# 92MING/Stable-Renderer

Hardware: AMD Instinct MI355X
Metric: frames/sec @512^2, SD1.5 20-step img2img, 8-view overlap (higher is better)
Workload: dtype f16

## Files before the change

include/sr_hip.h:

```cpp
#ifndef SR_HIP_H
#define SR_HIP_H
#include <stdint.h>
#ifdef __cplusplus
extern "C" {
#endif

typedef enum {
  SR_OK = 0,
  SR_ERR_INVALID = -1,
  SR_ERR_LAUNCH = -2,
  SR_ERR_UNSUPPORTED = -3
} sr_status;

typedef enum { SR_F16 = 0, SR_F32 = 1 } sr_dtype;

const char* sr_last_error(void);
int sr_version(void);
const char* sr_source_hash(void);
int sr_device_sync(void);

typedef struct {
  const void* a;
  const void* a2;
  const void* w;
  const float* bias;
  const float* rowvec;
  const void* residual;
  void* out;
  const void* zero_page;
  int32_t B, H, W;
  int32_t C1, C2;
  int32_t N;
  int32_t KH;
  int32_t stride;
  int32_t upsample;
  int32_t act;
  int32_t transpose_out;
  int32_t ldt;
  int32_t out_f32;
  int32_t dtype;
  float scale;
  int32_t rowvec_ld;
  void* workspace;
  int64_t workspace_bytes;
  const float* row_stats;
  const float* colsum;
  int32_t tile;
  int32_t split;
  int32_t pad_br;
  const void* prefetch;
  int64_t prefetch_bytes;
  int32_t up_h, up_w;
  int32_t* split_counters;
  int32_t group;
  int32_t ln_inline;
  float ln_eps;
  int32_t tile_order;
} sr_igemm_args;
#define SR_IGEMM_SPLIT_COUNTERS 4096
#define SR_IGEMM_GROUP_MAX 4
int sr_igemm(const sr_igemm_args* args, void* stream);
int sr_igemm_group(const sr_igemm_args* const* args, int32_t n, void* stream);

typedef struct {
  const void* x; const void* x2;
  const float* gamma; const float* beta;
  void* y;
  float* partials;
  int32_t B, HW, C1, C2, groups, silu, dtype;
  float eps;
} sr_groupnorm_args;
int sr_groupnorm(const sr_groupnorm_args* args, void* stream);
int64_t sr_groupnorm_scratch_floats(int32_t B, int32_t HW);

int sr_row_stats(const void* x, float* stats, int32_t rows, int32_t C, float eps, int32_t dtype, void* stream);
int sr_layernorm(const void* x, const float* gamma, const float* beta, void* y, int32_t rows, int32_t C,
                 float eps, int32_t dtype, void* stream);
int sr_layernorm_gather(const void* x, const int32_t* sel, int32_t nsel, int32_t frame_rows, int32_t n_frames, int32_t* err_flag,
                        const float* gamma, const float* beta, void* y, int32_t C, float eps, int32_t dtype, void* stream);

typedef struct {
  const void* q; const void* k; const void* vt; void* o;
  int32_t B, Bk, Tq, Tk, heads, d, ldt, dtype;
  int32_t q_stride, k_stride;
  float scale;
} sr_attention_args;
int sr_attention(const sr_attention_args* args, void* stream);

int sr_nchw_to_nhwc(const float* x, void* y, int32_t B, int32_t C, int32_t HW, int32_t Cpad, float scale_mul,
                    const float* per_batch_scale, int32_t dtype, void* stream);
int sr_nhwc_to_nchw(const void* x, float* y, int32_t B, int32_t C, int32_t HW, int32_t ldc, int32_t dtype,
                    void* stream);
int sr_timestep_embedding(const float* t, void* y, int32_t B, int32_t dim, int32_t dtype, void* stream);
int sr_silu(const void* x, void* y, int64_t n, int32_t dtype, void* stream);
int sr_cast(const void* x, int32_t src_dtype, void* y, int32_t dst_dtype, int64_t n, void* stream);
int sr_cache_touch(const void* p, int64_t bytes, void* stream);
int sr_softmax_rows(void* x, int32_t rows, int32_t cols, int32_t dtype, void* stream);
int sr_gather_rows(const void* x, const int32_t* sel, void* y, int32_t nsel, int32_t n_rows, int64_t row_bytes,
                   int32_t* err_flag, void* stream);
int sr_add_scaled(const void* a, const void* b, void* y, int64_t n, float s, int32_t dtype, void* stream);

typedef enum {
  SR_OP_IGEMM = 1, SR_OP_GROUPNORM = 2, SR_OP_LAYERNORM = 3, SR_OP_ATTENTION = 4, SR_OP_NCHW_TO_NHWC = 5,
  SR_OP_NHWC_TO_NCHW = 6, SR_OP_TIMESTEP_EMBED = 7, SR_OP_SILU = 8, SR_OP_SOFTMAX_ROWS = 9, SR_OP_GATHER_ROWS = 10, SR_OP_ADD_SCALED = 11,
  SR_OP_FORK = 12,
  SR_OP_JOIN = 13,
  SR_OP_ROW_STATS = 14,
  SR_OP_LAYERNORM_GATHER = 15
} sr_op_kind;
typedef struct {
  int32_t kind; int32_t lane;
  union {
    sr_igemm_args igemm;
    sr_groupnorm_args gn;
    sr_attention_args attn;
    struct { const void* x; const float* gamma; const float* beta; void* y; int32_t rows, C, dtype; float eps;
             const int32_t* sel; int32_t* err_flag; int32_t frame_rows, n_frames; } ln;
    struct { const void* x; void* y; const float* per_batch_scale; int32_t B, C, HW, Cpad, dtype, ldc; float scale; } cvt;
    struct { const float* t; void* y; int32_t B, dim, dtype; } temb;
    struct { const void* x; void* y; int64_t n; int32_t dtype; int32_t rows, cols; } ew;
    struct { const void* x; void* y; const int32_t* sel; int64_t row_bytes; int32_t nsel; int32_t n_rows; int32_t* err_flag; } gather;
    struct { const void* a; const void* b; void* y; int64_t n; float s; int32_t dtype; } add;
  } u;
} sr_op;
int sr_plan_run(const sr_op* host_ops, int32_t n_ops, void* stream);
int sr_plan_capture(const sr_op* host_ops, int32_t n_ops, void* stream, void** graph_exec);
int sr_graph_launch(void* graph_exec, void* stream);
int sr_graph_destroy(void* graph_exec);

typedef struct sr_model sr_model;
int sr_model_load(const char* path, sr_model** model);
int sr_model_free(sr_model* model);
int sr_model_io(sr_model* model, const char* name, void** dev_ptr, int64_t* nbytes);
int sr_model_run(sr_model* model, const char* plan, void* stream);
int sr_model_write(sr_model* model, const char* name, const void* src, void* stream);
int sr_model_read(sr_model* model, const char* name, void* dst, void* stream);
int sr_unet_forward(sr_model* unet, const float* x, const float* t, const void* ctx, float* out, void* stream);
int sr_vae_decode(sr_model* vae, const float* z, float* img, void* stream);

int sr_eps_scale_input(const float* x, float* xin, int64_t n_per_copy, int32_t copies, float sigma, void* stream);
int sr_cfg_denoise(const float* x, const float* eps, float* denoised, float* d, int64_t n, int32_t copies,
                   float sigma, float cfg, void* stream);
int sr_cond_crop_scale(const float* x, float* xin, int32_t N, int32_t C, int32_t h, int32_t w, int32_t ah, int32_t aw, int32_t y0,
                       int32_t x0, int32_t chunks, float sigma, void* stream);
int sr_cond_accumulate(const float* x, const float* eps, const float* mult, const int32_t* kinds, float* out_c, float* cnt_c,
// ... 88 lines not shown
```

stable-renderer_amd/_lib.py:

```python
import ctypes as C
import os

_HERE = os.path.dirname(os.path.abspath(__file__))
LIB_PATH = os.path.join(_HERE, "csrc", "libsr_hip.so")
_DEV_LIB = os.environ.get("SR_DEV_LIB")

SR_F16, SR_F32 = 0, 1
(OP_IGEMM, OP_GROUPNORM, OP_LAYERNORM, OP_ATTENTION, OP_NCHW_TO_NHWC, OP_NHWC_TO_NCHW, OP_TIMESTEP_EMBED, OP_SILU,
 OP_SOFTMAX_ROWS, OP_GATHER_ROWS, OP_ADD_SCALED, OP_FORK, OP_JOIN, OP_ROW_STATS, OP_LAYERNORM_GATHER) = range(1, 16)

vp = C.c_void_p
i32 = C.c_int32
i64 = C.c_int64
f32 = C.c_float


class IgemmArgs(C.Structure):
    _fields_ = [("a", vp), ("a2", vp), ("w", vp), ("bias", vp), ("rowvec", vp), ("residual", vp), ("out", vp),
                ("zero_page", vp), ("B", i32), ("H", i32), ("W", i32), ("C1", i32), ("C2", i32), ("N", i32),
                ("KH", i32), ("stride", i32), ("upsample", i32), ("act", i32), ("transpose_out", i32), ("ldt", i32),
                ("out_f32", i32), ("dtype", i32), ("scale", f32), ("rowvec_ld", i32), ("workspace", vp),
                ("workspace_bytes", C.c_int64), ("row_stats", vp), ("colsum", vp), ("tile", i32), ("split", i32), ("pad_br", i32),
                ("prefetch", vp), ("prefetch_bytes", C.c_int64), ("up_h", i32), ("up_w", i32), ("split_counters", vp), ("group", i32), ("ln_inline", i32), ("ln_eps", f32), ("tile_order", i32)]


class GroupNormArgs(C.Structure):
    _fields_ = [("x", vp), ("x2", vp), ("gamma", vp), ("beta", vp), ("y", vp), ("partials", vp), ("B", i32),
                ("HW", i32), ("C1", i32), ("C2", i32), ("groups", i32), ("silu", i32), ("dtype", i32), ("eps", f32)]


class AttentionArgs(C.Structure):
    _fields_ = [("q", vp), ("k", vp), ("vt", vp), ("o", vp), ("B", i32), ("Bk", i32), ("Tq", i32), ("Tk", i32),
                ("heads", i32), ("d", i32), ("ldt", i32), ("dtype", i32), ("q_stride", i32), ("k_stride", i32),
                ("scale", f32)]


class _Ln(C.Structure):
    _fields_ = [("x", vp), ("gamma", vp), ("beta", vp), ("y", vp), ("rows", i32), ("C", i32), ("dtype", i32), ("eps", f32),
                ("sel", vp), ("err_flag", vp), ("frame_rows", i32), ("n_frames", i32)]


class _Cvt(C.Structure):
    _fields_ = [("x", vp), ("y", vp), ("per_batch_scale", vp), ("B", i32), ("C", i32), ("HW", i32), ("Cpad", i32),
                ("dtype", i32), ("ldc", i32), ("scale", f32)]


class _Temb(C.Structure):
    _fields_ = [("t", vp), ("y", vp), ("B", i32), ("dim", i32), ("dtype", i32)]


class _Ew(C.Structure):
    _fields_ = [("x", vp), ("y", vp), ("n", i64), ("dtype", i32), ("rows", i32), ("cols", i32)]


class _Gather(C.Structure):
    _fields_ = [("x", vp), ("y", vp), ("sel", vp), ("row_bytes", i64), ("nsel", i32), ("n_rows", i32), ("err_flag", vp)]


class _Add(C.Structure):
    _fields_ = [("a", vp), ("b", vp), ("y", vp), ("n", i64), ("s", f32), ("dtype", i32)]


class _OpU(C.Union):
    _fields_ = [("igemm", IgemmArgs), ("gn", GroupNormArgs), ("attn", AttentionArgs), ("ln", _Ln), ("cvt", _Cvt),
                ("temb", _Temb), ("ew", _Ew), ("gather", _Gather), ("add", _Add)]


class Op(C.Structure):
    _fields_ = [("kind", i32), ("lane", i32), ("u", _OpU)]


class Draw(C.Structure):
    _fields_ = [("pos", vp), ("normal", vp), ("uv", vp), ("color", vp), ("vertex_id", vp), ("tris", vp), ("nv", i32),
                ("nt", i32), ("MV", f32 * 16), ("MV_IT", f32 * 16), ("P", f32 * 16), ("sprite_id", i32),
                ("material_id", i32), ("corrmap_k", i32), ("use_texcoord_id", i32), ("render_mode", i32),
                ("has_vertex_color", i32), ("depth_test", i32), ("cull_back", i32), ("id_w", i32), ("id_h", i32),
                ("noise_tex", vp), ("noise_w", i32), ("noise_h", i32), ("diffuse_tex", vp), ("diffuse_w", i32),
                ("diffuse_h", i32), ("corrmap_tex", vp), ("corr_w", i32), ("corr_h", i32),
                ("tangent", vp), ("bitangent", vp), ("normal_tex", vp), ("normal_w", i32), ("normal_h", i32), ("diffuse_levels", i32)]


class GBuffer(C.Structure):
    _fields_ = [("color", vp), ("id", vp), ("pos", vp), ("normal_depth", vp), ("noise", vp), ("canny", vp), ("zbuf", vp),
                ("W", i32), ("H", i32)]


P = C.POINTER
SYMBOLS = {
    "sr_last_error": (C.c_char_p, []),
    "sr_version": (C.c_int, []),
    "sr_source_hash": (C.c_char_p, []),
    "sr_device_sync": (C.c_int, []),
    "sr_model_load": (C.c_int, [C.c_char_p, P(vp)]),
    "sr_model_free": (C.c_int, [vp]),
    "sr_model_io": (C.c_int, [vp, C.c_char_p, P(vp), P(i64)]),
    "sr_model_run": (C.c_int, [vp, C.c_char_p, vp]),
    "sr_model_write": (C.c_int, [vp, C.c_char_p, vp, vp]),
    "sr_model_read": (C.c_int, [vp, C.c_char_p, vp, vp]),
    "sr_unet_forward": (C.c_int, [vp, vp, vp, vp, vp, vp]),
    "sr_vae_decode": (C.c_int, [vp, vp, vp, vp]),
    "sr_layernorm_gather": (C.c_int, [vp, vp, i32, i32, i32, vp, vp, vp, vp, i32, f32, i32, vp]),
    "sr_igemm": (C.c_int, [P(IgemmArgs), vp]),
    "sr_igemm_group": (C.c_int, [P(P(IgemmArgs)), i32, vp]),
    "sr_groupnorm": (C.c_int, [P(GroupNormArgs), vp]),
    "sr_groupnorm_scratch_floats": (i64, [i32, i32]),
    "sr_layernorm": (C.c_int, [vp, vp, vp, vp, i32, i32, f32, i32, vp]),
    "sr_row_stats": (C.c_int, [vp, vp, i32, i32, f32, i32, vp]),
    "sr_attention": (C.c_int, [P(AttentionArgs), vp]),
    "sr_nchw_to_nhwc": (C.c_int, [vp, vp, i32, i32, i32, i32, f32, vp, i32, vp]),
    "sr_nhwc_to_nchw": (C.c_int, [vp, vp, i32, i32, i32, i32, i32, vp]),
    "sr_timestep_embedding": (C.c_int, [vp, vp, i32, i32, i32, vp]),
    "sr_silu": (C.c_int, [vp, vp, i64, i32, vp]),
    "sr_cast": (C.c_int, [vp, i32, vp, i32, i64, vp]),
    "sr_cache_touch": (C.c_int, [vp, i64, vp]),
    "sr_softmax_rows": (C.c_int, [vp, i32, i32, i32, vp]),
    "sr_gather_rows": (C.c_int, [vp, vp, vp, i32, i32, i64, vp, vp]),
    "sr_add_scaled": (C.c_int, [vp, vp, vp, i64, f32, i32, vp]),
    "sr_plan_run": (C.c_int, [P(Op), i32, vp]),
    "sr_plan_capture": (C.c_int, [P(Op), i32, vp, P(vp)]),
    "sr_graph_launch": (C.c_int, [vp, vp]),
    "sr_graph_destroy": (C.c_int, [vp]),
    "sr_eps_scale_input": (C.c_int, [vp, vp, i64, i32, f32, vp]),
    "sr_cfg_denoise": (C.c_int, [vp, vp, vp, vp, i64, i32, f32, f32, vp]),
    "sr_cond_crop_scale": (C.c_int, [vp, vp, i32, i32, i32, i32, i32, i32, i32, i32, i32, f32, vp]),
    "sr_cond_accumulate": (C.c_int, [vp, vp, vp, vp, vp, vp, vp, vp, i32, i32, i32, i32, i32, i32, i32, i32, i32, f32, vp]),
    "sr_cfg_combine": (C.c_int, [vp, vp, vp, vp, vp, vp, vp, i64, f32, f32, vp]),
    "sr_euler_step": (C.c_int, [vp, vp, i64, f32, vp]),
    "sr_vae_sample": (C.c_int, [vp, vp, vp, i32, i32, i32, vp]),
    "sr_ddpm_step": (C.c_int, [vp, vp, vp, i64, f32, f32, vp]),
    "sr_lcm_step": (C.c_int, [vp, vp, vp, i64, f32, vp]),
    "sr_axpby": (C.c_int, [vp, vp, i64, f32, f32, vp]),
    "sr_idmap_masks": (C.c_int, [vp, vp, i64, vp]),
    "sr_overlap_build": (C.c_int, [vp, i32, i32, i32, i32, i32, vp, vp, vp, vp]),
    "sr_overlap_csr_scratch_ints": (i64, [i32]),
    "sr_overlap_csr": (C.c_int, [vp, vp, i32, i32, i32, i32, vp, vp, vp, vp]),
    "sr_overlap_step": (C.c_int, [vp, vp, vp, vp, i32, i32, i32, i32, i32, f32, vp, vp]),
    "sr_legacy_overlap": (C.c_int, [vp, vp, vp, vp, vp, vp, vp, vp, i32, i32, i32, i32, i32, i32, f32, i32, i32, i32, vp]),
    "sr_legacy_levels": (C.c_int, [vp, vp, vp, vp, vp, i32, i32, i32, i32, i32, vp, vp]),
    "sr_legacy_overlap_seq": (C.c_int, [vp, vp, vp, vp, i32, i32, vp, vp, vp, vp, vp, i32, i32, i32, f32, i32, i32, vp]),
    "sr_nearest_resize": (C.c_int, [vp, vp, i64, i32, i32, i32, i32, vp, vp]),
    "sr_adain": (C.c_int, [vp, i64, i64, i64, i32, vp, i32, i64, i64, i64, i32, vp, i32, i32, f32, vp, vp]),
    "sr_noise_pool": (C.c_int, [vp, vp, vp, vp, vp, i32, i32, vp, vp]),
    "sr_noise_pool_strips": (C.c_int, [vp, vp, vp, vp, vp, i32, i32, i32, vp, vp]),
    "sr_corrmap_update": (C.c_int, [vp, i32, vp, vp, vp, i32, i32, i32, i32, i32, i32, vp, vp, i32, i32, vp, vp, vp]),
    "sr_gbuffer_clear": (C.c_int, [P(GBuffer), vp]),
    "sr_gbuffer_depth_merge": (C.c_int, [P(GBuffer), P(GBuffer), vp]),
    "sr_defer_post": (C.c_int, [vp, vp, vp, i32, i32, i32, i32, i32, f32, f32, f32, f32, f32, vp]),
    "sr_raster_draw": (C.c_int, [P(Draw), P(GBuffer), vp, i64, vp]),
    "sr_raster_scratch_bytes": (i64, [i32, i32, i32]),
}

_lib = None


class SrHipError(RuntimeError):
    pass


def _build_module():
    import importlib.util
    spec = importlib.util.spec_from_file_location("sr_build", os.path.join(_HERE, "csrc", "build.py"))
    mod = importlib.util.module_from_spec(spec)
    spec.loader.exec_module(mod)
    return mod


def _load():
    L = C.CDLL(LIB_PATH)
    for name, (res, args) in SYMBOLS.items():
        fn = getattr(L, name)
        fn.restype = res
        fn.argtypes = args
    return L


def lib():
    global _lib
    if _lib is None and _DEV_LIB:
        L = C.CDLL(_DEV_LIB)
        for name, (res, args) in SYMBOLS.items():
            fn = getattr(L, name)
            fn.restype = res
            fn.argtypes = args
        _lib = L
    if _lib is None:
        bm = _build_module()
# ... 48 lines not shown
```

stable-renderer_amd/csrc/build.py:

```python
import os
import subprocess
import sys
from concurrent.futures import ThreadPoolExecutor

HERE = os.path.dirname(os.path.abspath(__file__))
OBJ = os.path.join(HERE, "_obj")
LIB = os.path.join(HERE, "libsr_hip.so")
SOURCES = ["errors.cpp", "hostutil.cpp", "model.cpp", "igemm.hip", "norm.hip", "attention.hip", "eltwise.hip", "overlap.hip", "plan.hip", "raster.hip"]
FLAGS = ["--offload-arch=gfx950", "-O3", "-std=c++17", "-fPIC"]
EXTRA = {"raster.hip": ["-ffp-contract=off"],
         "attention.hip": ["-fno-honor-nans"]}
HEADERS = ["sr_common.h", os.path.join("..", "..", "include", "sr_hip.h")]


def hipcc():
    for c in (os.environ.get("HIPCC"), "/opt/rocm/bin/hipcc", "hipcc"):
        if c and (os.path.isabs(c) and os.path.exists(c) or not os.path.isabs(c)):
            return c
    raise RuntimeError("hipcc not found")


def source_hash():
    import hashlib
    h = hashlib.sha256()
    for f in sorted(SOURCES) + sorted(HEADERS) + [os.path.basename(__file__)]:
        fp = os.path.join(HERE, f)
        if os.path.exists(fp):
            h.update(f.encode())
            with open(fp, "rb") as fh:
                h.update(fh.read())
    return h.hexdigest()[:32]


def _needs(src, obj):
    if not os.path.exists(obj):
        return True
    t = os.path.getmtime(obj)
    deps = [os.path.join(HERE, src), os.path.abspath(__file__)] + [os.path.join(HERE, h) for h in HEADERS]
    return any(os.path.getmtime(d) > t for d in deps)


def build(force=False, verbose=False):
    os.makedirs(OBJ, exist_ok=True)
    cc = hipcc()
    srcs = [s for s in SOURCES if os.path.exists(os.path.join(HERE, s))]
    jobs = []
    sh = source_hash()
    stamp = os.path.join(OBJ, "src.hash")
    stale_stamp = not os.path.exists(stamp) or open(stamp).read().strip() != sh
    for s in srcs:
        obj = os.path.join(OBJ, os.path.splitext(s)[0] + ".o")
        if force or _needs(s, obj) or (s == "errors.cpp" and stale_stamp):
            cmd = [cc] + FLAGS + EXTRA.get(s, []) + ([f'-DSR_SRC_HASH="{sh}"'] if s == "errors.cpp" else []) + (["-x", "hip"] if s.endswith(".cpp") else []) + ["-c", os.path.join(HERE, s), "-o", obj]
            jobs.append((s, cmd))

    def run(job):
        s, cmd = job
        r = subprocess.run(cmd, capture_output=True, text=True)
        if r.returncode != 0:
            raise RuntimeError("hipcc failed for %s:\n%s" % (s, r.stderr[-4000:]))
        if verbose:
            print("compiled", s)
    with ThreadPoolExecutor(max_workers=4) as ex:
        list(ex.map(run, jobs))
    objs = [os.path.join(OBJ, os.path.splitext(s)[0] + ".o") for s in srcs]
    if jobs or not os.path.exists(LIB):
        tmp = LIB + ".tmp%d" % os.getpid()
        r = subprocess.run([cc, "--offload-arch=gfx950", "-shared", "-fPIC", "-o", tmp] + objs, capture_output=True, text=True)
        if r.returncode != 0:
            if os.path.exists(tmp):
                os.unlink(tmp)
            raise RuntimeError("link failed:\n" + r.stderr[-4000:])
        os.replace(tmp, LIB)
    with open(stamp, "w") as f:
        f.write(sh)
    return LIB


def built_hash():
    stamp = os.path.join(OBJ, "src.hash")
    if os.path.exists(LIB) and os.path.exists(stamp):
        return open(stamp).read().strip()
    return None


if __name__ == "__main__":
    print(build(force="--force" in sys.argv, verbose=True))
```

stable-renderer_amd/csrc/igemm.hip:

```cpp
#include "sr_common.h"
#ifndef SR_IGEMM_TRACE
#define SR_IGEMM_TRACE 0
#endif
#if SR_IGEMM_TRACE
#define SR_TS(k) do { if (threadIdx.x == 0) ts_[k] = wall_clock64(); } while (0)
#else
#define SR_TS(k) do { } while (0)
#endif
#include <stdlib.h>
#include <type_traits>

namespace {

#define SR_FOLD(p) ((p).row_stats != nullptr || (p).ln_inline != 0)
__device__ __forceinline__ float2 sr_fold_stat(const sr_igemm_args& p, const int m, const int m0) {
  extern __shared__ __attribute__((aligned(16))) char sr_lds_front[];
  if (p.ln_inline) return *(const float2*)(sr_lds_front + 8 * (m - m0));
  return *(const float2*)(p.row_stats + 2 * (int64_t)m);
}

template <typename T, int BM, int BN, int WAVES_M, int WAVES_N, int LDS_AVAIL, bool GEGLU, int VCAP, bool VECPRE>
__device__ __forceinline__ void epilogue_rows_h(const sr_igemm_args& p, f32x4 (&acc)[BN / WAVES_N / 16][BM / WAVES_M / 16], char* smem, const int M,
                                                const int rpb, const int m0, const int n0, const int pm0, const int qn0, const int wv,
                                                const int lane) {
// ... 973 lines not shown
  const int NT = a.N / 320, nwg = (M / 256) * NT;
  static bool attr_set = false;
  if (!attr_set) { (void)hipFuncSetAttribute((const void*)conv3p_kernel, hipFuncAttributeMaxDynamicSharedMemorySize, lds); attr_set = true; }
  hipLaunchKernelGGL(conv3p_kernel, dim3(nwg), dim3(512), lds, st, a, M, NT, nwg);
  SR_CHECK_LAUNCH("sr_igemm(conv3p)");
  return SR_OK;
}

static inline int plan_split(int64_t tiles, int KT, int slots, double t_k, int64_t tile_ws_bytes, int64_t ws_bytes, int* tile0, int forceS = 0) {
  const int64_t full = tiles / slots, tail = tiles - full * slots;
  *tile0 = (int)(full * slots);
  if (tail == 0) return 1;
  if (forceS > 0)
    return (KT / forceS >= 4 && (int64_t)forceS * tail * tile_ws_bytes <= ws_bytes) ? forceS : -1;
  if (const char* fs = getenv("SR_SPLIT_S")) {
    const int S = atoi(fs);
    if (S >= 1 && KT / S >= 4 && (int64_t)S * tail * tile_ws_bytes <= ws_bytes) return S;
  }
  double best = (double)KT * t_k;
  int bestS = 1;
  for (int S = 2; S <= 16; ++S) {
    if (KT / S < 8 || (int64_t)S * tail * tile_ws_bytes > ws_bytes) break;
    const int64_t rounds = (tail * S + slots - 1) / slots;
    const double t = (double)rounds * ((KT + S - 1) / S) * t_k + (double)(2 * S * tail * tile_ws_bytes) / 4.0e6 + 14.0;
    if (t < best * 0.9) { best = t; bestS = S; }
  }
  return bestS;
}

template <typename T, bool TRANS>
int dispatch(const sr_igemm_args& a, int M, int Ho, int Wo, hipStream_t st) {
  const int n128 = (a.N + 127) / 128, n64 = (a.N + 63) / 64;
  const int64_t wg_128x128 = (int64_t)((M + 127) / 128) * n128;
  const bool waste128 = (n128 * 128 - a.N) * 8 > a.N;
  const char* fenv = getenv("SR_IGEMM_TILE");
  const int force = fenv ? atoi(fenv) : a.tile;
  static const bool split_off = getenv("SR_SPLITK") && atoi(getenv("SR_SPLITK")) == 0;
  const int KT = a.KH * a.KH * ((a.C1 + a.C2) / (int)(128 / sizeof(T)));
  const int forceS = a.split > 1 ? a.split : 0;
  const bool can_split = !TRANS && !split_off && a.split >= 0 && a.workspace && a.act != 2 && a.N % 4 == 0 && !a.ln_inline;
  const bool may_split = can_split && KT >= 32;
  const bool deep_split = can_split && KT >= 8 && (force == 14 || force == 15);
  if (forceS && !((may_split && (force == 2 || force == 3)) || deep_split))
    SR_FAIL(SR_ERR_INVALID, "sr_igemm: split = %d needs tile 2 / 3 (K >= 32 steps) or 14 / 15 (K >= 8 steps), a workspace, no GEGLU / transposed output", a.split);
  if constexpr (!TRANS) {
    if (deep_split && forceS) {
      int tile0 = 0;
      const int64_t tiles = force == 15 ? wg_128x128 : (int64_t)((M + 127) / 128) * n64;
      const int S = plan_split(tiles, KT, 256, 1.0, 128 * (force == 15 ? 128 : 64) * 4, a.workspace_bytes, &tile0, forceS);
      if (S < 0) SR_FAIL(SR_ERR_INVALID, "sr_igemm: split = %d does not fit this shape (K steps %d, workspace %lld B)", a.split, KT, (long long)a.workspace_bytes);
      if (S > 1) return force == 15 ? launch_split<T, 128, 128, 4>(a, M, Ho, Wo, tile0, S, st) : launch_split<T, 128, 64, 6>(a, M, Ho, Wo, tile0, S, st);
      SR_FAIL(SR_ERR_INVALID, "sr_igemm: split = %d: nothing to split (whole rounds of workgroups only)", a.split);
    }
    if (may_split && (force == 2 || force == 3)) {
      int tile0 = 0;
      if (force == 2) {
        const int S = plan_split(wg_128x128, KT, 512, 1.2, 128 * 128 * 4, a.workspace_bytes, &tile0, forceS);
        if (S < 0) SR_FAIL(SR_ERR_INVALID, "sr_igemm: split = %d does not fit this shape (K steps %d, workspace %lld B)", a.split, KT, (long long)a.workspace_bytes);
        if (S > 1) return launch_split<T, 128, 128>(a, M, Ho, Wo, tile0, S, st);
      } else {
        const int S = plan_split((int64_t)((M + 127) / 128) * n64, KT, 768, 0.93, 128 * 64 * 4, a.workspace_bytes, &tile0, forceS);
        if (S < 0) SR_FAIL(SR_ERR_INVALID, "sr_igemm: split = %d does not fit this shape (K steps %d, workspace %lld B)", a.split, KT, (long long)a.workspace_bytes);
        if (S > 1) return launch_split<T, 128, 64>(a, M, Ho, Wo, tile0, S, st);
      }
      if (forceS) SR_FAIL(SR_ERR_INVALID, "sr_igemm: split = %d: nothing to split (whole rounds of workgroups only)", a.split);
    }
  }
  if (force == 2) return launch_ln<T, 128, 128, 2, 2, 2, TRANS>(a, M, Ho, Wo, st);
  if (force == 3) return launch_ln<T, 128, 64, 2, 2, 2, TRANS>(a, M, Ho, Wo, st);
  if (force == 4) return launch_ln<T, 64, 64, 2, 2, 2, TRANS>(a, M, Ho, Wo, st);
  if (force == 13) return launch_ln<T, 64, 64, 2, 2, 8, TRANS>(a, M, Ho, Wo, st);
  if (force == 14) return launch_ln<T, 128, 64, 2, 2, 6, TRANS>(a, M, Ho, Wo, st);
  if (force == 15) return launch_ln<T, 128, 128, 2, 2, 4, TRANS>(a, M, Ho, Wo, st);
  if (force == 8) {
    if constexpr (!TRANS && sizeof(T) == 2) { if (conv3p_ok(a, M)) return launch_conv3p(a, M, st); }
    SR_FAIL(SR_ERR_INVALID, "sr_igemm: tile 8 (patch-stationary 3x3) needs fp16, KH=3, stride 1, one source, N %% 320 == 0, "
                            "256-pixel tiles of whole rows / images (H=%d W=%d M=%d N=%d)", a.H, a.W, M, a.N);
  }
  if constexpr (!TRANS && sizeof(T) == 2) {
    if ((force >= 5 && force <= 7) && a.N % 320) SR_FAIL(SR_ERR_INVALID, "sr_igemm: tile %d (256x320) needs N %% 320 == 0, N=%d", force, a.N);
    if (force == 6) return launch<T, 256, 320, 4, 2, 4, TRANS, 64>(a, M, Ho, Wo, st);
    if (force == 9) {
      if (a.N % 160) SR_FAIL(SR_ERR_INVALID, "sr_igemm: tile 9 (128x160) needs N %% 160 == 0, N=%d", a.N);
      return launch_ln<T, 128, 160, 4, 2, 2, TRANS, 128, 0, 4>(a, M, Ho, Wo, st);
    }
    if (force == 10) {
      if (a.N % 320) SR_FAIL(SR_ERR_INVALID, "sr_igemm: tile 10 (128x320) needs N %% 320 == 0, N=%d", a.N);
      return launch_ln<T, 128, 320, 2, 4, 2, TRANS, 64, 0, 4>(a, M, Ho, Wo, st);
    }
    if (force == 11) return launch_ln<T, 128, 128, 4, 2, 2, TRANS, 128, 0, 4>(a, M, Ho, Wo, st);
    if (force == 12) return launch_ln<T, 256, 128, 4, 2, 2, TRANS, 64, 0, 4>(a, M, Ho, Wo, st);
    if (force == 7 || (force == 0 && a.N % 320 == 0 && (int64_t)((M + 255) / 256) * (a.N / 320) < 256 &&
                       (int64_t)((M + 127) / 128) * (a.N / 320) >= 256))
      return launch_ln<T, 128, 320, 2, 4, 2, TRANS>(a, M, Ho, Wo, st);

    if (force == 5 || (force == 0 && a.N % 320 == 0 && (int64_t)((M + 255) / 256) * (a.N / 320) >= 256))
      return launch_ln<T, 256, 320, 4, 2, 2, TRANS, 128, 2>(a, M, Ho, Wo, st);
  } else {
    if (force >= 5 && force <= 12) SR_FAIL(SR_ERR_INVALID, "sr_igemm: tile %d is fp16, non-transposed only", force);
  }
  const int64_t wg_256x128 = (int64_t)((M + 255) / 256) * n128;
  const bool big = !waste128 && wg_256x128 >= 512;
  if constexpr (!TRANS) {
    if (force == 0 && may_split && !big) {
      int tile0 = 0;
      if (!waste128) {
        const int S = plan_split(wg_128x128, KT, 512, 1.2, 128 * 128 * 4, a.workspace_bytes, &tile0);
        if (S > 1) return launch_split<T, 128, 128>(a, M, Ho, Wo, tile0, S, st);
      } else {
        const int S = plan_split((int64_t)((M + 127) / 128) * n64, KT, 768, 0.93, 128 * 64 * 4, a.workspace_bytes, &tile0);
        if (S > 1) return launch_split<T, 128, 64>(a, M, Ho, Wo, tile0, S, st);
      }
    }
  }
  if (force == 1 || (force == 0 && big && !a.ln_inline))
    return launch<T, 256, 128, 4, 2, 3, TRANS, 128, 1>(a, M, Ho, Wo, st);
  if (!waste128 && wg_128x128 >= 192 && !(a.KH == 1 && wg_128x128 <= 768)) return launch_ln<T, 128, 128, 2, 2, 2, TRANS>(a, M, Ho, Wo, st);
  const int64_t wg_128x64 = (int64_t)((M + 127) / 128) * n64;
  if (wg_128x64 >= 192) return launch_ln<T, 128, 64, 2, 2, 2, TRANS>(a, M, Ho, Wo, st);
  if ((int64_t)((M + 63) / 64) * n64 <= 256 && KT >= 4) return launch_ln<T, 64, 64, 2, 2, 8, TRANS>(a, M, Ho, Wo, st);
  return launch_ln<T, 64, 64, 2, 2, 2, TRANS>(a, M, Ho, Wo, st);
}

}

static int igemm_check(const sr_igemm_args* a, int* M_, int* Ho_, int* Wo_) {
  if (!a || !a->a || !a->w || !a->out || !a->zero_page) SR_FAIL(SR_ERR_INVALID, "sr_igemm: null pointer");
  const int ke = a->dtype == SR_F16 ? 64 : 32;
  if (a->dtype != SR_F16 && a->dtype != SR_F32) SR_FAIL(SR_ERR_INVALID, "sr_igemm: bad dtype %d", a->dtype);
  if (a->C1 <= 0 || a->C1 % ke || a->C2 % ke || a->C2 < 0) SR_FAIL(SR_ERR_INVALID, "sr_igemm: C1=%d C2=%d must be multiples of %d", a->C1, a->C2, ke);
  if (a->C2 > 0 && !a->a2) SR_FAIL(SR_ERR_INVALID, "sr_igemm: C2>0 without a2");
  if (a->KH != 1 && a->KH != 3) SR_FAIL(SR_ERR_INVALID, "sr_igemm: KH=%d", a->KH);
  if (a->stride != 1 && a->stride != 2) SR_FAIL(SR_ERR_INVALID, "sr_igemm: stride=%d", a->stride);
  if (a->upsample && a->stride != 1) SR_FAIL(SR_ERR_INVALID, "sr_igemm: upsample with stride");
  if (a->pad_br && (a->KH != 3 || a->upsample)) SR_FAIL(SR_ERR_INVALID, "sr_igemm: pad_br is for 3x3 convs without upsample");
  if (a->N <= 0 || a->B <= 0 || a->H <= 0 || a->W <= 0) SR_FAIL(SR_ERR_INVALID, "sr_igemm: bad sizes");
  if (a->act == 2 && (a->N % 4 || a->transpose_out)) SR_FAIL(SR_ERR_INVALID, "sr_igemm: GEGLU needs N%%4==0");
  if (a->row_stats && !a->colsum) SR_FAIL(SR_ERR_INVALID, "sr_igemm: row_stats without colsum");
  if (a->ln_inline && (a->row_stats || !a->colsum)) SR_FAIL(SR_ERR_INVALID, "sr_igemm: ln_inline takes colsum and no row_stats");
  if ((a->row_stats || a->ln_inline) && (a->KH != 1 || a->stride != 1 || a->upsample || a->C2)) SR_FAIL(SR_ERR_INVALID, "sr_igemm: folded LayerNorm is for 1x1 single-source layers");
  if (a->tile < 0 || a->tile > 15 || a->split < -1 || a->split == 1 || a->split > 16) SR_FAIL(SR_ERR_INVALID, "sr_igemm: tile=%d split=%d", a->tile, a->split);
  if (a->tile_order != 0 && a->tile_order != 1) SR_FAIL(SR_ERR_INVALID, "sr_igemm: tile_order=%d (0 rows first, 1 columns first)", a->tile_order);
  int Ho, Wo;
  if (a->upsample && ((a->up_h > 0) != (a->up_w > 0))) SR_FAIL(SR_ERR_INVALID, "sr_igemm: up_h / up_w go together");
  if (!a->upsample && (a->up_h || a->up_w)) SR_FAIL(SR_ERR_INVALID, "sr_igemm: up_h / up_w without upsample");
  if (a->upsample) { Ho = a->up_h > 0 ? a->up_h : 2 * a->H; Wo = a->up_w > 0 ? a->up_w : 2 * a->W; }
  else if (a->stride == 2) {
    const int ptot = a->pad_br ? a->KH / 2 : 2 * (a->KH / 2);
    Ho = (a->H + ptot - a->KH) / 2 + 1; Wo = (a->W + ptot - a->KH) / 2 + 1;
  }
  else { Ho = a->H; Wo = a->W; }
  const int64_t M64 = (int64_t)a->B * Ho * Wo;
  if (M64 > 0x7fffffffLL / 2) SR_FAIL(SR_ERR_INVALID, "sr_igemm: M too large");
  if (a->transpose_out && a->ldt < Ho * Wo) SR_FAIL(SR_ERR_INVALID, "sr_igemm: ldt < pixels per batch");
  *M_ = (int)M64; *Ho_ = Ho; *Wo_ = Wo;
  return SR_OK;
}

extern "C" int sr_igemm(const sr_igemm_args* a, void* stream) {
  int M, Ho, Wo;
  const int rc = igemm_check(a, &M, &Ho, &Wo);
  if (rc != SR_OK) return rc;
  hipStream_t st = sr_stream(stream);
  if (a->dtype == SR_F16) {
    return a->transpose_out ? dispatch<_Float16, true>(*a, M, Ho, Wo, st) : dispatch<_Float16, false>(*a, M, Ho, Wo, st);
  }
  return a->transpose_out ? dispatch<float, true>(*a, M, Ho, Wo, st) : dispatch<float, false>(*a, M, Ho, Wo, st);
}

template <typename T>
static int group_launch(int tile, const sr_igemm_args* const* as, const int* Ms, const int* Hos, const int* Wos, int n, hipStream_t st) {
  switch (tile) {
    case 2: return launch_group<T, 128, 128, 2, 2, 2>(as, Ms, Hos, Wos, n, st);
    case 3: return launch_group<T, 128, 64, 2, 2, 2>(as, Ms, Hos, Wos, n, st);
    case 4: return launch_group<T, 64, 64, 2, 2, 2>(as, Ms, Hos, Wos, n, st);
    case 13: return launch_group<T, 64, 64, 2, 2, 8>(as, Ms, Hos, Wos, n, st);
    case 14: return launch_group<T, 128, 64, 2, 2, 6>(as, Ms, Hos, Wos, n, st);
    case 15: return launch_group<T, 128, 128, 2, 2, 4>(as, Ms, Hos, Wos, n, st);
    default: break;
  }
// ... 32 lines not shown
```

stable-renderer_amd/csrc/sr_common.h:

```cpp
#pragma once
#include <hip/hip_runtime.h>
#include <hip/hip_fp16.h>
#include <stdint.h>
#include <stdio.h>
#include <stdarg.h>
#include "../../include/sr_hip.h"

typedef float f32x4 __attribute__((ext_vector_type(4)));
typedef float f32x2 __attribute__((ext_vector_type(2)));
typedef _Float16 h16x8 __attribute__((ext_vector_type(8)));
typedef _Float16 h16x4 __attribute__((ext_vector_type(4)));
typedef _Float16 h16x2 __attribute__((ext_vector_type(2)));

void sr_set_error(const char* fmt, ...);
#define SR_FAIL(code, ...) do { sr_set_error(__VA_ARGS__); return (code); } while (0)
#define SR_CHECK_LAUNCH(name) do { hipError_t e_ = hipGetLastError(); if (e_ != hipSuccess) { \
    sr_set_error("%s: %s", name, hipGetErrorString(e_)); return SR_ERR_LAUNCH; } } while (0)

template <typename T> struct sr_traits;
template <> struct sr_traits<_Float16> { static constexpr int EPC = 8;   };
template <> struct sr_traits<float>    { static constexpr int EPC = 4; };

__device__ __forceinline__ void sr_mma(f32x4& acc, const uint4& a, const uint4& b, _Float16) {
  acc = __builtin_amdgcn_mfma_f32_16x16x32_f16(__builtin_bit_cast(h16x8, a), __builtin_bit_cast(h16x8, b), acc, 0, 0, 0);
}
__device__ __forceinline__ void sr_mma(f32x4& acc, const uint4& a, const uint4& b, float) {
  acc = __builtin_amdgcn_mfma_f32_16x16x4f32(__uint_as_float(a.x), __uint_as_float(b.x), acc, 0, 0, 0);
  acc = __builtin_amdgcn_mfma_f32_16x16x4f32(__uint_as_float(a.y), __uint_as_float(b.y), acc, 0, 0, 0);
  acc = __builtin_amdgcn_mfma_f32_16x16x4f32(__uint_as_float(a.z), __uint_as_float(b.z), acc, 0, 0, 0);
  acc = __builtin_amdgcn_mfma_f32_16x16x4f32(__uint_as_float(a.w), __uint_as_float(b.w), acc, 0, 0, 0);
}

__device__ __forceinline__ void sr_glds16(const void* gsrc, void* lds_wave_base) {
  __builtin_amdgcn_global_load_lds((const __attribute__((address_space(1))) void*)gsrc,
                                   (__attribute__((address_space(3))) void*)lds_wave_base, 16, 0, 0);
}

__device__ __forceinline__ void sr_glds16_asm(const void* gsrc, unsigned lds_addr) {
  unsigned keep;
  asm volatile("s_mov_b32 %0, m0\n\ts_mov_b32 m0, %2\n\ts_nop 0\n\tglobal_load_lds_dwordx4 %1, off\n\ts_mov_b32 m0, %0"
               : "=&s"(keep) : "v"(gsrc), "s"(lds_addr) : "memory");
}
__device__ __forceinline__ unsigned sr_m0_save() {
  unsigned keep;
  asm volatile("s_mov_b32 %0, m0" : "=s"(keep));
  return keep;
}
__device__ __forceinline__ void sr_m0_restore(unsigned keep) { asm volatile("s_mov_b32 m0, %0" ::"s"(keep)); }
__device__ __forceinline__ void sr_glds16_asm_nosave(const void* gsrc, unsigned lds_addr) {
  asm volatile("s_mov_b32 m0, %1\n\ts_nop 0\n\tglobal_load_lds_dwordx4 %0, off" ::"v"(gsrc), "s"(lds_addr) : "memory");
}
__device__ __forceinline__ void sr_glds16_asm_saddr(unsigned voff, const void* sbase, unsigned lds_addr) {
  asm volatile("s_mov_b32 m0, %2\n\ts_nop 0\n\tglobal_load_lds_dwordx4 %0, %1" ::"v"(voff), "s"(sbase), "s"(lds_addr) : "memory");
}
__device__ __forceinline__ void sr_prefetch_touch(const void* base, int64_t bytes, int64_t gtid, int64_t gthreads, unsigned lds_scratch_wave) {
  const int64_t n = bytes >> 6;
  const unsigned keep = sr_m0_save();
  for (int64_t i = gtid; i < n; i += gthreads) {
    const char* src = (const char*)base + (i << 6);
    asm volatile("s_mov_b32 m0, %1\n\ts_nop 0\n\tglobal_load_lds_dword %0, off" ::"v"(src), "s"(lds_scratch_wave) : "memory");
  }
  sr_m0_restore(keep);
}
__device__ __forceinline__ unsigned sr_lds_addr(const void* p) {
  return (unsigned)(size_t)(__attribute__((address_space(3))) const char*)p;
}

__device__ __forceinline__ float sr_silu_f(float x) { return x / (1.0f + __expf(-x)); }
__device__ __forceinline__ float sr_gelu_f(float x) {
  const float z = fabsf(x) * 0.70710678118654752440f;
  const float t = __builtin_amdgcn_rcpf(fmaf(0.3275911f, z, 1.0f));
  float poly = fmaf(1.061405429f, t, -1.453152027f);
  poly = fmaf(poly, t, 1.421413741f);
  poly = fmaf(poly, t, -0.284496736f);
  poly = fmaf(poly, t, 0.254829592f);
  const float e = poly * t * __expf(-z * z);
  const float cdf = x >= 0.0f ? 1.0f - 0.5f * e : 0.5f * e;
  return x * cdf;
}

__device__ __forceinline__ float sr_load_f(const _Float16* p) { return (float)*p; }
__device__ __forceinline__ float sr_load_f(const float* p) { return *p; }
__device__ __forceinline__ void sr_store_f(_Float16* p, float v) { *p = (_Float16)v; }
__device__ __forceinline__ void sr_store_f(float* p, float v) { *p = v; }

__device__ __forceinline__ int sr_xcd_remap(int bid, int nwg) {
  const int q = nwg >> 3, r = nwg & 7, xcd = bid & 7, loc = bid >> 3;
  return (xcd < r ? xcd * (q + 1) : r * (q + 1) + (xcd - r) * q) + loc;
}

__device__ __forceinline__ void sr_tile_of(int wg, int NT, int MT, int order, int& mt, int& nt) {
  if (order == 1) { nt = wg / MT; mt = wg - nt * MT; }
  else            { mt = wg / NT; nt = wg - mt * NT; }
}

static inline hipStream_t sr_stream(void* s) { return (hipStream_t)s; }
static inline int sr_cdiv(int64_t a, int64_t b) { return (int)((a + b - 1) / b); }
```

Before: 22.00.

## Add persistent weight-stationary streaming kernel for small-K fp16 linear layers

Adds a persistent kernel for 1x1 fp16 GEMMs with K up to 320 and N a multiple of 160. Each block loads a 160-column weight slice into swizzled LDS once, then walks a contiguous strip of 32-row blocks with register-prefetched activations, fusing bias, rowvec and residual into the epilogue. It is routed from the igemm dispatcher for tiles 9, 10 and 5 and the default large-N path, and aims to cut repeated weight loads and tile-scheduling overhead on tall, skinny projections. The grid size is derived from the CU count, which can leave load imbalance. Eligibility is narrow, and it can be disabled with an environment variable.

```diff
diff --git a/include/sr_hip.h b/include/sr_hip.h
--- a/include/sr_hip.h
+++ b/include/sr_hip.h
@@ -61,6 +61,9 @@
 #define SR_IGEMM_GROUP_MAX 4
 int sr_igemm(const sr_igemm_args* args, void* stream);
 int sr_igemm_group(const sr_igemm_args* const* args, int32_t n, void* stream);
+int sr_linear_stream_eligible(const sr_igemm_args* args);
+int64_t sr_linear_stream_min_rows(int32_t N);
+int64_t sr_linear_stream_launch_count(void);
 
 typedef struct {
   const void* x; const void* x2;
diff --git a/stable-renderer_amd/_lib.py b/stable-renderer_amd/_lib.py
--- a/stable-renderer_amd/_lib.py
+++ b/stable-renderer_amd/_lib.py
@@ -102,6 +102,9 @@
     "sr_layernorm_gather": (C.c_int, [vp, vp, i32, i32, i32, vp, vp, vp, vp, i32, f32, i32, vp]),
     "sr_igemm": (C.c_int, [P(IgemmArgs), vp]),
     "sr_igemm_group": (C.c_int, [P(P(IgemmArgs)), i32, vp]),
+    "sr_linear_stream_eligible": (C.c_int, [P(IgemmArgs)]),
+    "sr_linear_stream_min_rows": (i64, [i32]),
+    "sr_linear_stream_launch_count": (i64, []),
     "sr_groupnorm": (C.c_int, [P(GroupNormArgs), vp]),
     "sr_groupnorm_scratch_floats": (i64, [i32, i32]),
     "sr_layernorm": (C.c_int, [vp, vp, vp, vp, i32, i32, f32, i32, vp]),
diff --git a/stable-renderer_amd/csrc/build.py b/stable-renderer_amd/csrc/build.py
--- a/stable-renderer_amd/csrc/build.py
+++ b/stable-renderer_amd/csrc/build.py
@@ -6,11 +6,11 @@
 HERE = os.path.dirname(os.path.abspath(__file__))
 OBJ = os.path.join(HERE, "_obj")
 LIB = os.path.join(HERE, "libsr_hip.so")
-SOURCES = ["errors.cpp", "hostutil.cpp", "model.cpp", "igemm.hip", "norm.hip", "attention.hip", "eltwise.hip", "overlap.hip", "plan.hip", "raster.hip"]
+SOURCES = ["errors.cpp", "hostutil.cpp", "model.cpp", "igemm.hip", "linear_stream.hip", "norm.hip", "attention.hip", "eltwise.hip", "overlap.hip", "plan.hip", "raster.hip"]
 FLAGS = ["--offload-arch=gfx950", "-O3", "-std=c++17", "-fPIC"]
 EXTRA = {"raster.hip": ["-ffp-contract=off"],
          "attention.hip": ["-fno-honor-nans"]}
-HEADERS = ["sr_common.h", os.path.join("..", "..", "include", "sr_hip.h")]
+HEADERS = ["sr_common.h", "linear_stream.h", os.path.join("..", "..", "include", "sr_hip.h")]
 
 
 def hipcc():
diff --git a/stable-renderer_amd/csrc/igemm.hip b/stable-renderer_amd/csrc/igemm.hip
--- a/stable-renderer_amd/csrc/igemm.hip
+++ b/stable-renderer_amd/csrc/igemm.hip
@@ -1079,10 +1079,12 @@
     if (force == 6) return launch<T, 256, 320, 4, 2, 4, TRANS, 64>(a, M, Ho, Wo, st);
     if (force == 9) {
       if (a.N % 160) SR_FAIL(SR_ERR_INVALID, "sr_igemm: tile 9 (128x160) needs N %% 160 == 0, N=%d", a.N);
+      if (sr_linear_stream_takes(a, M)) return sr_linear_stream_launch(a, M, Ho * Wo, st);
       return launch_ln<T, 128, 160, 4, 2, 2, TRANS, 128, 0, 4>(a, M, Ho, Wo, st);
     }
     if (force == 10) {
       if (a.N % 320) SR_FAIL(SR_ERR_INVALID, "sr_igemm: tile 10 (128x320) needs N %% 320 == 0, N=%d", a.N);
+      if (sr_linear_stream_takes(a, M)) return sr_linear_stream_launch(a, M, Ho * Wo, st);
       return launch_ln<T, 128, 320, 2, 4, 2, TRANS, 64, 0, 4>(a, M, Ho, Wo, st);
     }
     if (force == 11) return launch_ln<T, 128, 128, 4, 2, 2, TRANS, 128, 0, 4>(a, M, Ho, Wo, st);
@@ -1091,8 +1093,10 @@
                        (int64_t)((M + 127) / 128) * (a.N / 320) >= 256))
       return launch_ln<T, 128, 320, 2, 4, 2, TRANS>(a, M, Ho, Wo, st);
 
-    if (force == 5 || (force == 0 && a.N % 320 == 0 && (int64_t)((M + 255) / 256) * (a.N / 320) >= 256))
+    if (force == 5 || (force == 0 && a.N % 320 == 0 && (int64_t)((M + 255) / 256) * (a.N / 320) >= 256)) {
+      if (sr_linear_stream_takes(a, M)) return sr_linear_stream_launch(a, M, Ho * Wo, st);
       return launch_ln<T, 256, 320, 4, 2, 2, TRANS, 128, 2>(a, M, Ho, Wo, st);
+    }
   } else {
     if (force >= 5 && force <= 12) SR_FAIL(SR_ERR_INVALID, "sr_igemm: tile %d is fp16, non-transposed only", force);
   }
diff --git a/stable-renderer_amd/csrc/linear_stream.h b/stable-renderer_amd/csrc/linear_stream.h
--- /dev/null
+++ b/stable-renderer_amd/csrc/linear_stream.h
@@ -0,0 +1,50 @@
+#pragma once
+#include <stdint.h>
+#include "../../include/sr_hip.h"
+#if defined(__HIPCC__)
+#define SR_LS_HD __host__ __device__
+#else
+#define SR_LS_HD
+#endif
+
+enum {
+  SR_LS_BN = 160,
+  SR_LS_ROWS = 32,
+  SR_LS_WAVES = 8,
+  SR_LS_KMAX = 320,
+  SR_LS_MIN_BLOCKS = 4
+};
+
+static inline SR_LS_HD int sr_ls_strips(int N, int cus) {
+  const int halves = N / SR_LS_BN;
+  if (halves < 1 || N % SR_LS_BN) return 0;
+  return (cus / halves) / 8 * 8;
+}
+
+static inline SR_LS_HD void sr_ls_tile_of(int b, int halves, int* strip, int* half) {
+  const int xcd = b & 7, loc = b >> 3;
+  *half = loc % halves;
+  *strip = (loc / halves) * 8 + xcd;
+}
+
+static inline SR_LS_HD void sr_ls_strip_blocks(int M, int strips, int s, int* lo, int* hi) {
+  const int64_t nb = ((int64_t)M + SR_LS_ROWS - 1) / SR_LS_ROWS;
+  *lo = (int)(nb * s / strips);
+  *hi = (int)(nb * (s + 1) / strips);
+}
+
+static inline SR_LS_HD int64_t sr_ls_min_rows(int N, int cus) {
+  return (int64_t)sr_ls_strips(N, cus) * SR_LS_MIN_BLOCKS * SR_LS_ROWS;
+}
+
+static inline int sr_ls_eligible(const sr_igemm_args* a, int64_t M, int cus) {
+  if (a->dtype != SR_F16 || a->KH != 1 || a->stride != 1 || a->upsample || a->C2 != 0 || a->transpose_out) return 0;
+  if (a->act != 0 || a->out_f32 || a->split != -1) return 0;
+  if (a->scale != 1.0f) return 0;
+  if (a->row_stats || a->ln_inline) return 0;
+  if (a->C1 <= 0 || a->C1 > SR_LS_KMAX || a->C1 % 64) return 0;
+  if (a->N <= 0 || a->N % SR_LS_BN) return 0;
+  const int strips = sr_ls_strips(a->N, cus);
+  if (strips < 8) return 0;
+  return M >= sr_ls_min_rows(a->N, cus) && M <= 0x3fffffff;
+}
diff --git a/stable-renderer_amd/csrc/linear_stream.hip b/stable-renderer_amd/csrc/linear_stream.hip
--- /dev/null
+++ b/stable-renderer_amd/csrc/linear_stream.hip
@@ -0,0 +1,216 @@
+#include "sr_common.h"
+#include "linear_stream.h"
+#include <stdlib.h>
+
+#include <atomic>
+
+namespace {
+
+std::atomic<int64_t> ls_launches{0};
+constexpr int LS_PF_B = SR_LS_WAVES * 256;
+constexpr int LS_VEC_B = SR_LS_BN * 4;
+
+template <int NJ, bool RES, bool RV>
+__global__ __launch_bounds__(SR_LS_WAVES * 64, 2) void linear_stream_kernel(const sr_igemm_args p, const int M, const int rpb,
+                                                                            const int strips, const int halves) {
+  extern __shared__ __attribute__((aligned(16))) char ls_smem[];
+  constexpr int K = NJ * 32, KB = K * 2;
+  constexpr int R = NJ == 10 ? 5 : (NJ == 8 ? 4 : NJ);
+  constexpr int TN = SR_LS_BN / 16, TM = SR_LS_ROWS / 16, NP = TN / 2;
+  constexpr int WSTEP = SR_LS_BN * 128;
+  static_assert(NJ % 2 == 0 && NJ % R == 0 && K <= SR_LS_KMAX, "K is whole 64-half steps, at most 320");
+  float* const lbias = (float*)(ls_smem + LS_PF_B);
+  char* const lw = ls_smem + LS_PF_B + LS_VEC_B;
+
+  const int tid = threadIdx.x, lane = tid & 63;
+  const int wv = __builtin_amdgcn_readfirstlane(tid >> 6);
+  const int c16 = lane & 15, g4 = lane >> 4;
+  if (p.prefetch)
+    sr_prefetch_touch(p.prefetch, p.prefetch_bytes, (int64_t)blockIdx.x * (SR_LS_WAVES * 64) + tid, (int64_t)gridDim.x * (SR_LS_WAVES * 64),
+                      __builtin_amdgcn_readfirstlane(sr_lds_addr(ls_smem) + wv * 256));
+  int strip, half, b_lo, b_hi;
+  sr_ls_tile_of(blockIdx.x, halves, &strip, &half);
+  sr_ls_strip_blocks(M, strips, strip, &b_lo, &b_hi);
+  const int n0 = half * SR_LS_BN;
+  const int N = p.N;
+
+  const char* const X = (const char*)p.a + g4 * 16;
+  auto xrow = [&](int blk, int t) {
+    const int m = blk * SR_LS_ROWS + t * 16 + c16;
+    return X + (int64_t)(m < M ? m : M - 1) * KB;
+  };
+  int blk = b_lo + wv;
+  uint4 xf[R][TM];
+  if (blk < b_hi) {
+    const char* r0 = xrow(blk, 0);
+    const char* r1 = xrow(blk, 1);
+#pragma unroll
+    for (int j = 0; j < R; ++j) { xf[j][0] = *(const uint4*)(r0 + j * 64); xf[j][1] = *(const uint4*)(r1 + j * 64); }
+  }
+
+  {
+    constexpr int CPR = K / 8;
+    const char* const Wg = (const char*)p.w;
+    constexpr int NCH = SR_LS_BN * CPR, NIT = (NCH + SR_LS_WAVES * 64 - 1) / (SR_LS_WAVES * 64);
+    uint4 wv4[NIT];
+    int wdst[NIT];
+#pragma unroll
+    for (int it = 0; it < NIT; ++it) {
+      const int c0 = it * (SR_LS_WAVES * 64) + tid, c = c0 < NCH ? c0 : NCH - 1;
+      const int lr = c / CPR, ch = c - lr * CPR;
+      const int tn = lr >> 4, i = lr & 15;
+      const int n = n0 + (tn >> 1) * 32 + (i >> 2) * 8 + (tn & 1) * 4 + (i & 3);
+      wv4[it] = *(const uint4*)(Wg + (int64_t)n * KB + ch * 16);
+      wdst[it] = (ch >> 3) * WSTEP + lr * 128 + (((ch & 7) ^ (lr & 7)) << 4);
+    }
+#pragma unroll
+    for (int it = 0; it < NIT; ++it) *(uint4*)(lw + wdst[it]) = wv4[it];
+    if (tid < SR_LS_BN) lbias[tid] = p.bias ? p.bias[n0 + tid] : 0.f;
+  }
+  __syncthreads();
+
+  const bool has_bias = p.bias != nullptr;
+  const int ldr = p.rowvec_ld ? p.rowvec_ld : N;
+  const int foff0 = c16 * 128 + (((0 + g4) ^ (c16 & 7)) << 4), foff1 = c16 * 128 + (((4 + g4) ^ (c16 & 7)) << 4);
+  const int ncol = n0 + g4 * 8;
+
+  while (blk < b_hi) {
+    const int nblk = blk + SR_LS_WAVES;
+    const bool more = nblk < b_hi;
+    const char* const rc0 = xrow(blk, 0);
+    const char* const rc1 = xrow(blk, 1);
+    const char* const rn0 = more ? xrow(nblk, 0) : (const char*)p.a;
+    const char* const rn1 = more ? xrow(nblk, 1) : (const char*)p.a;
+    int fo0 = foff0, fo1 = foff1;
+    asm volatile("" : "+v"(fo0), "+v"(fo1));
+    uint4 rr[RES ? TM : 1][RES ? NP : 1];
+    if constexpr (RES) {
+#pragma unroll
+      for (int tm = 0; tm < TM; ++tm) {
+        const int m = blk * SR_LS_ROWS + tm * 16 + c16;
+        const _Float16* const rrow = (const _Float16*)p.residual + (int64_t)(m < M ? m : M - 1) * N + ncol;
+#pragma unroll
+        for (int q = 0; q < NP; ++q) rr[tm][q] = *(const uint4*)(rrow + q * 32);
+      }
+    }
+    __builtin_amdgcn_sched_barrier(0);
+    f32x4 acc[TN][TM];
+#pragma unroll
+    for (int tn = 0; tn < TN; ++tn)
+#pragma unroll
+      for (int tm = 0; tm < TM; ++tm) acc[tn][tm] = f32x4{0.f, 0.f, 0.f, 0.f};
+#pragma unroll
+    for (int j = 0; j < NJ; ++j) {
+      const char* wb = lw + (j >> 1) * WSTEP + ((j & 1) ? fo1 : fo0);
+      uint4 wf[TN];
+#pragma unroll
+      for (int tn = 0; tn < TN; ++tn) wf[tn] = *(const uint4*)(wb + tn * (16 * 128));
+#pragma unroll
+      for (int tn = 0; tn < TN; ++tn)
+#pragma unroll
+        for (int tm = 0; tm < TM; ++tm) sr_mma(acc[tn][tm], wf[tn], xf[j % R][tm], _Float16());
+      const int jn = j + R;
+      if (jn < NJ) {
+        xf[j % R][0] = *(const uint4*)(rc0 + jn * 64);
+        xf[j % R][1] = *(const uint4*)(rc1 + jn * 64);
+      } else {
+        xf[j % R][0] = *(const uint4*)(rn0 + (jn - NJ) * 64);
+        xf[j % R][1] = *(const uint4*)(rn1 + (jn - NJ) * 64);
+      }
+      __builtin_amdgcn_sched_barrier(0);
+    }
+#pragma unroll
+    for (int tm = 0; tm < TM; ++tm) {
+      const int m = blk * SR_LS_ROWS + tm * 16 + c16;
+      const bool valid = m < M;
+      const int b = (RV && valid) ? m / rpb : 0;
+#pragma unroll
+      for (int q = 0; q < NP; ++q) {
+        h16x8 hv;
+#pragma unroll
+        for (int h = 0; h < 2; ++h) {
+          const int tn = 2 * q + h;
+          const int nl = q * 32 + g4 * 8 + h * 4;
+          float v[4] = {acc[tn][tm][0], acc[tn][tm][1], acc[tn][tm][2], acc[tn][tm][3]};
+          {
+            const float4 bv = *(const float4*)(lbias + nl);
+            v[0] = has_bias ? v[0] + bv.x : v[0]; v[1] = has_bias ? v[1] + bv.y : v[1];
+            v[2] = has_bias ? v[2] + bv.z : v[2]; v[3] = has_bias ? v[3] + bv.w : v[3];
+          }
+          if constexpr (RV) { const float4 rv = *(const float4*)(p.rowvec + (int64_t)b * ldr + n0 + nl); v[0] += rv.x; v[1] += rv.y; v[2] += rv.z; v[3] += rv.w; }
+          hv[h * 4 + 0] = (_Float16)v[0]; hv[h * 4 + 1] = (_Float16)v[1]; hv[h * 4 + 2] = (_Float16)v[2]; hv[h * 4 + 3] = (_Float16)v[3];
+        }
+        if constexpr (RES) {
+          const h16x8 r8 = __builtin_bit_cast(h16x8, rr[tm][q]);
+#pragma unroll
+          for (int e = 0; e < 8; ++e) hv[e] = (_Float16)((float)hv[e] + (float)r8[e]);
+        }
+        if (valid) *(uint4*)((_Float16*)p.out + (int64_t)m * N + ncol + q * 32) = __builtin_bit_cast(uint4, hv);
+      }
+    }
+    blk = nblk;
+  }
+}
+
+template <int NJ, bool RES, bool RV>
+int launch_impl(const sr_igemm_args& a, int M, int rpb, int strips, int halves, hipStream_t st) {
+  const int lds = LS_PF_B + LS_VEC_B + SR_LS_BN * NJ * 64;
+  auto k = linear_stream_kernel<NJ, RES, RV>;
+  static bool attr_set = false;
+  if (!attr_set) { (void)hipFuncSetAttribute((const void*)k, hipFuncAttributeMaxDynamicSharedMemorySize, lds); attr_set = true; }
+  hipLaunchKernelGGL(k, dim3(strips * halves), dim3(SR_LS_WAVES * 64), lds, st, a, M, rpb, strips, halves);
+  SR_CHECK_LAUNCH("sr_igemm(linear stream)");
+  ls_launches.fetch_add(1, std::memory_order_relaxed);
+  return SR_OK;
+}
+
+template <int NJ>
+int launch_nj(const sr_igemm_args& a, int M, int rpb, int strips, int halves, hipStream_t st) {
+  if (a.residual) return a.rowvec ? launch_impl<NJ, true, true>(a, M, rpb, strips, halves, st) : launch_impl<NJ, true, false>(a, M, rpb, strips, halves, st);
+  return a.rowvec ? launch_impl<NJ, false, true>(a, M, rpb, strips, halves, st) : launch_impl<NJ, false, false>(a, M, rpb, strips, halves, st);
+}
+
+}
+
+int sr_linear_stream_cus() {
+  static int cached[64];
+  int dev = 0;
+  if (hipGetDevice(&dev) != hipSuccess || dev < 0 || dev >= 64) return 0;
+  if (cached[dev] == 0) {
+    int n = 0;
+    if (hipDeviceGetAttribute(&n, hipDeviceAttributeMultiprocessorCount, dev) != hipSuccess) return 0;
+    cached[dev] = n;
+  }
+  return cached[dev];
+}
+
+bool sr_linear_stream_takes(const sr_igemm_args& a, int M) {
+  const char* e = getenv("SR_LINEAR_STREAM");
+  if (e && atoi(e) == 0) return false;
+  return sr_ls_eligible(&a, M, sr_linear_stream_cus()) != 0;
+}
+
+int sr_linear_stream_launch(const sr_igemm_args& a, int M, int rpb, hipStream_t st) {
+  const int cus = sr_linear_stream_cus();
+  const int halves = a.N / SR_LS_BN, strips = sr_ls_strips(a.N, cus);
+  if (!sr_ls_eligible(&a, M, cus)) SR_FAIL(SR_ERR_INVALID, "sr_igemm: the linear stream kernel does not take this call");
+  switch (a.C1 / 32) {
+    case 2: return launch_nj<2>(a, M, rpb, strips, halves, st);
+    case 4: return launch_nj<4>(a, M, rpb, strips, halves, st);
+    case 6: return launch_nj<6>(a, M, rpb, strips, halves, st);
+    case 8: return launch_nj<8>(a, M, rpb, strips, halves, st);
+    case 10: return launch_nj<10>(a, M, rpb, strips, halves, st);
+    default: break;
+  }
+  SR_FAIL(SR_ERR_INVALID, "sr_igemm: the linear stream kernel needs C1 in {64, 128, 192, 256, 320}, C1=%d", a.C1);
+}
+
+extern "C" int sr_linear_stream_eligible(const sr_igemm_args* a) {
+  if (!a || a->B <= 0 || a->H <= 0 || a->W <= 0) return 0;
+  const int64_t M = (int64_t)a->B * a->H * a->W;
+  return sr_ls_eligible(a, M, sr_linear_stream_cus());
+}
+
+extern "C" int64_t sr_linear_stream_launch_count(void) { return ls_launches.load(std::memory_order_relaxed); }
+
+extern "C" int64_t sr_linear_stream_min_rows(int32_t N) { return sr_ls_min_rows(N, sr_linear_stream_cus()); }
diff --git a/stable-renderer_amd/csrc/sr_common.h b/stable-renderer_amd/csrc/sr_common.h
--- a/stable-renderer_amd/csrc/sr_common.h
+++ b/stable-renderer_amd/csrc/sr_common.h
@@ -94,5 +94,8 @@
   else            { mt = wg / NT; nt = wg - mt * NT; }
 }
 
+bool sr_linear_stream_takes(const sr_igemm_args& a, int M);
+int sr_linear_stream_launch(const sr_igemm_args& a, int M, int rpb, hipStream_t st);
+
 static inline hipStream_t sr_stream(void* s) { return (hipStream_t)s; }
 static inline int sr_cdiv(int64_t a, int64_t b) { return (int)((a + b - 1) / b); }
```

New measurement: 21.99. No clear change (-0.1%).
